# baresip/re

Hardware: AMD Instinct MI355X
Metric: GiB/s + Mpkt/s SRTP protect+unprotect, 1200B RTP pkts, device-resident (higher is better)
Workload: dtype u8

## Files before the change

re_amd/csrc/hip/k_ctr_fast.h:

```cpp
#pragma once
#include "kern_common.h"

#ifndef CTRF_BLOCK
#define CTRF_BLOCK 1024
#endif
#ifndef CTRF_BLOCK_U
#define CTRF_BLOCK_U CTRF_BLOCK
#endif
#define CTRF_BLK(PROT) ((PROT) ? CTRF_BLOCK : CTRF_BLOCK_U)
#ifndef CTRF_COAL_P
#define CTRF_COAL_P 1
#endif
#ifndef CTRF_COAL_U
#define CTRF_COAL_U 1
#endif
#ifndef CTRF_COAL_MK
#define CTRF_COAL_MK 1
#endif
#ifndef CTRF_SB_ST
#define CTRF_SB_ST 0
#endif
#ifndef CTRF_PRIO
#define CTRF_PRIO 0
#endif
#ifndef CTRF_SHAFIRST_U
#define CTRF_SHAFIRST_U 1
#endif
#ifndef CTRF_SB_BLOCKS
#define CTRF_SB_BLOCKS 0
#endif
#ifndef CTRF_SB_SHA
#define CTRF_SB_SHA 0
#endif

template <int NR, int SHIFT>
__device__ __forceinline__ void fast_ks_xor(const uint8_t *smem, uint32_t lo,
					    const uint32_t *rk,
					    const CtrKs<NR, true, true> &C,
					    int32_t blk0, uint32_t carry[4],
					    uint32_t d[16])
{
#pragma unroll
	for (int q = 0; q < SHIFT; q++)
		d[q] ^= carry[4 - SHIFT + q];
#pragma unroll
	for (int m = 0; m < 4; m++) {
		uint32_t B[4];
		C.block(smem, lo, rk, blk0 + m, B);
#pragma unroll
		for (int q = 0; q < 4; q++) {
			const int jj = SHIFT + 4 * m + q;
			if (jj < 16)
				d[jj] ^= B[q];
			else
				carry[q] = B[q];
		}
		if (m == 3 && SHIFT == 0) {
#pragma unroll
			for (int q = 0; q < 4; q++)
				carry[q] = B[q];
		}
		if (CTRF_SB_BLOCKS && (m + 1) % (CTRF_SB_BLOCKS > 0 ?
						 CTRF_SB_BLOCKS : 1) == 0 &&
		    m < 3)
			__builtin_amdgcn_sched_barrier(0);
	}
}

struct FastPkt {
	uint32_t p, off, L, hl, ssrc, ixhi, ixlo, roc;
};

template <bool RTCP = false>
__device__ __forceinline__ bool fast_pkt(const struct sgpu_compact &c,
					 uint32_t t, FastPkt &f)
{
	if (t >= c.n)
		return false;
	f.p = c.idx ? c.idx[c.base + t] : c.base + t;
	const uint64_t d = c.desc[f.p];
	const uint32_t fl = (uint32_t)(d >> 48);
	if (!(fl & SD_RUN))
		return false;
	f.off = c.pos[f.p];
	f.L = c.end[f.p] - f.off;
	const uint32_t *hw = (const uint32_t *)(c.hdr + f.p);
	f.ssrc = hw[0];
	f.hl = hw[2];
	if (RTCP) {
		const uint32_t w = (uint32_t)d;
		f.ixhi = (w & 0x7fffffffu) >> 16;
		f.ixlo = w & 0xffffu;
		f.roc = w;
		return true;
	}
	f.ixhi = (uint32_t)(d >> 16);
	f.ixlo = (uint32_t)(d & 0xffffu);
	f.roc = f.ixhi + ((fl & SD_ROC_P1) ? 1u : 0u) -
		((fl & SD_ROC_M1) ? 1u : 0u);
	return true;
}

template <int NR>
__device__ __forceinline__ const struct sgpu_comp *
fast_keys_at(const KArgs &a, uint32_t ci, uint32_t rk[4 * (NR + 1)])
{
	const struct sgpu_comp *cp = a.comps + ci;
#pragma unroll
	for (int k = 0; k < NR + 1; k++) {
		const uint4 v = *(const uint4 *)&cp->rk[4 * k];
		rk[4 * k] = v.x; rk[4 * k + 1] = v.y;
		rk[4 * k + 2] = v.z; rk[4 * k + 3] = v.w;
	}
#pragma unroll
	for (int k = 4; k < 4 * NR; k++)
		rk[k] = rot16(rk[k]);
#pragma unroll
	for (int k = 0; k < 4 * (NR + 1); k++)
		rk[k] = __builtin_amdgcn_readfirstlane(rk[k]);
	return cp;
}

template <int NR>
__device__ __forceinline__ const struct sgpu_comp *
fast_keys(const KArgs &a, uint32_t rk[4 * (NR + 1)])
{
	return fast_keys_at<NR>(
		a, __builtin_amdgcn_readfirstlane(a.c.compmap[0]), rk);
}

template <int NR>
__device__ __forceinline__ const struct sgpu_comp *
lane_keys(const KArgs &a, const FastPkt &f, uint32_t rk[4 * (NR + 1)])
{
	const struct sgpu_comp *cp = a.comps + a.c.compmap[a.c.sess[f.p]];
#pragma unroll
	for (int k = 0; k < NR + 1; k++) {
		const uint4 v = *(const uint4 *)&cp->rk[4 * k];
		rk[4 * k] = v.x; rk[4 * k + 1] = v.y;
		rk[4 * k + 2] = v.z; rk[4 * k + 3] = v.w;
	}
#pragma unroll
	for (int k = 4; k < 4 * NR; k++)
		rk[k] = rot16(rk[k]);
	return cp;
}

__device__ __forceinline__ void fast_iv(const struct sgpu_comp *cp,
					const FastPkt &f, uint32_t iv[4])
{
	const uint4 ks = *(const uint4 *)cp->k_s;
	iv[0] = ks.x;
	iv[1] = ks.y ^ bswap32(f.ssrc);
	iv[2] = ks.z ^ bswap32(f.ixhi);
	iv[3] = (ks.w ^ (bswap32(f.ixlo) >> 16)) & 0xffffu;
}

template <int NR, int SHIFT>
__device__ __forceinline__ void tail_xor_store(const uint8_t *smem,
					       uint32_t lo, const uint32_t *rk,
					       const CtrKs<NR, true, true> &C,
					       int32_t blk0, uint32_t carry[4],
					       uint32_t d[16], uint8_t *pkt,
					       uint32_t c0, uint32_t c_off,
					       uint32_t c_end)
{
	uint32_t ks[16];
	chunk_ks<NR, SHIFT>(smem, lo, rk, C, blk0, carry, ks);
#pragma unroll
	for (int jj = 0; jj < 16; jj++) {
		const uint32_t bpos = c0 + 4u * jj;
		uint32_t m = region_mask(bpos, c_off, c_end);
		asm volatile("" : "+v"(m));
		d[jj] = __builtin_amdgcn_bitop3_b32(d[jj], ks[jj], m, 0x78);
		if (bpos + 4u > c_off && bpos < c_end)
			*(uint32_t *)(pkt + bpos) = d[jj];
	}
}

template <int NR, int SHIFT, bool PROT, bool MK = false, bool RTCP = false>
__device__ __forceinline__ void ctr_fast_pkt(const KArgs &a, uint8_t *smem,
					     const FastPkt &f, uint32_t ci)
{
	uint32_t rk[4 * (NR + 1)];
	const struct sgpu_comp *cp = MK ? lane_keys<NR>(a, f, rk)
					: fast_keys_at<NR>(a, ci, rk);
	const uint32_t lo = (threadIdx.x & 31u) * 4u;
	const uint32_t lane = threadIdx.x & 63u;
	uint8_t *const arena = a.arena;
	uint8_t *const pkt = arena + f.off;
	const uint64_t pasz = a.asz - f.off;
	const uint32_t T = PROT ? 0u : __builtin_amdgcn_readfirstlane(cp->tag_len);
	const uint32_t A = f.L - T - (RTCP && !PROT ? 4u : 0u);
	const uint32_t hl = RTCP && !(f.roc >> 31) ? A : f.hl;

	uint32_t iv[4];
	fast_iv(cp, f, iv);
	CtrKs<NR, true, true> C;
	C.init(smem, lo, rk, iv);
	uint32_t h[5] = {cp->ipad[0], cp->ipad[1], cp->ipad[2], cp->ipad[3],
			 cp->ipad[4]};
	const uint64_t X = (uint64_t)f.roc << 32 | 0x80000000u;
	const uint32_t nb = (A + 4u + 9u + 63u) / 64u;
	const uint64_t bitlen = (uint64_t)(64u + A + 4u) * 8u;
	const int32_t cw4 = (int32_t)(hl >> 4);
	const uint32_t kf0 = hl < 16u ? 0u : min((hl + 63u) / 64u, nb);
	const uint32_t kf1 = max(A / 64u, kf0);
	uint32_t carry[4] = {0, 0, 0, 0};

	auto general = [&](uint32_t k) {
		const uint32_t c0 = 64u * k;
		uint32_t d[16], w[16];
#pragma unroll
		for (int g = 0; g < 4; g++) {
			uint4 v = make_uint4(0, 0, 0, 0);
			if (c0 + 16u * g < A)
				v = ld16(pkt, pasz, c0 + 16u * g);
			d[4 * g] = v.x; d[4 * g + 1] = v.y;
			d[4 * g + 2] = v.z; d[4 * g + 3] = v.w;
		}
		if (!PROT) {
#pragma unroll
			for (int jj = 0; jj < 16; jj++)
				w[jj] = msg_word(16u * k + jj, bswap32(d[jj]), A, X);
		}
		if (c0 + 64u > hl && c0 < A)
			tail_xor_store<NR, SHIFT>(smem, lo, rk, C,
						  (int32_t)(4 * k) - cw4, carry,
						  d, pkt, c0, hl, A);
		if (PROT) {
#pragma unroll
			for (int jj = 0; jj < 16; jj++)
				w[jj] = msg_word(16u * k + jj, bswap32(d[jj]), A, X);
		}
		if (k + 1 == nb) {
			w[14] = (uint32_t)(bitlen >> 32);
			w[15] = (uint32_t)bitlen;
		}
		sha1_compress(h, w);
	};

	uint32_t k = 0;
	for (; k < kf0; k++)
		general(k);

	constexpr bool COAL = MK ? CTRF_COAL_MK :
			      PROT ? CTRF_COAL_P : CTRF_COAL_U;
	uint32_t K0 = kf1, K1 = kf1;
	uint32_t qo[4];
	if constexpr (COAL) {
		qo[0] = qdpp<0x00>(f.off) + 16u * (lane & 3u);
		qo[1] = qdpp<0x55>(f.off) + 16u * (lane & 3u);
		qo[2] = qdpp<0xAA>(f.off) + 16u * (lane & 3u);
		qo[3] = qdpp<0xFF>(f.off) + 16u * (lane & 3u);
		const uint64_t act = __ballot(1);
		uint32_t a0 = max(kf0, qdpp<DPP_QXOR1>(kf0));
		a0 = max(a0, qdpp<DPP_QXOR2>(a0));
		uint32_t a1 = min(kf1, qdpp<DPP_QXOR1>(kf1));
		a1 = min(a1, qdpp<DPP_QXOR2>(a1));
		if (((act >> (lane & ~3u)) & 0xfull) == 0xfull && a0 < a1) {
			K0 = a0;
			K1 = a1;
		}
	}
	auto steady = [&](uint32_t k, auto coal) {
		constexpr bool CO = decltype(coal)::value;
		const uint32_t c0 = 64u * k;
		if (CTRF_PRIO) {
			const uint32_t q4 =
				(uint32_t)__builtin_amdgcn_readfirstlane(4u * k) /
				(uint32_t)__builtin_amdgcn_readfirstlane(nb);
			if (q4 == 0)
				__builtin_amdgcn_s_setprio(3);
			else if (q4 == 1)
				__builtin_amdgcn_s_setprio(2);
			else if (q4 == 2)
				__builtin_amdgcn_s_setprio(1);
			else
				__builtin_amdgcn_s_setprio(0);
		}
		uint32_t d[16], w[16];
		if constexpr (CO) {
			uint32_t x[4][4];
#pragma unroll
			for (int g = 0; g < 4; g++) {
				const uint4 v = *(const uint4 *)(arena + (qo[g] + c0));
				x[g][0] = v.x; x[g][1] = v.y; x[g][2] = v.z;
				x[g][3] = v.w;
			}
			quad_transpose(x, lane);
#pragma unroll
			for (int q = 0; q < 4; q++)
#pragma unroll
				for (int cc = 0; cc < 4; cc++)
					d[4 * q + cc] = x[q][cc];
		}
		else {
#pragma unroll
			for (int g = 0; g < 4; g++) {
				const uint4 v = *(const uint4 *)(pkt + c0 + 16u * g);
				d[4 * g] = v.x; d[4 * g + 1] = v.y;
				d[4 * g + 2] = v.z; d[4 * g + 3] = v.w;
			}
		}
		if (!PROT && CTRF_SHAFIRST_U) {
#pragma unroll
			for (int jj = 0; jj < 16; jj++)
				w[jj] = bswap32(d[jj]);
			sha1_compress(h, w);
			if (CTRF_SB_SHA)
				__builtin_amdgcn_sched_barrier(0);
		}
		fast_ks_xor<NR, SHIFT>(smem, lo, rk, C, (int32_t)(4 * k) - cw4,
				       carry, d);
		if constexpr (CO) {
			uint32_t x[4][4];
#pragma unroll
			for (int q = 0; q < 4; q++)
#pragma unroll
				for (int cc = 0; cc < 4; cc++)
					x[q][cc] = d[4 * q + cc];
			quad_transpose(x, lane);
#pragma unroll
			for (int g = 0; g < 4; g++)
				*(uint4 *)(arena + (qo[g] + c0)) =
					make_uint4(x[g][0], x[g][1], x[g][2],
						   x[g][3]);
		}
		else {
			if (CTRF_SB_ST)
				__builtin_amdgcn_sched_barrier(0);
#pragma unroll
			for (int g = 0; g < 4; g++)
				*(uint4 *)(pkt + c0 + 16u * g) =
					make_uint4(d[4 * g], d[4 * g + 1],
						   d[4 * g + 2], d[4 * g + 3]);
		}
		if (PROT) {
#pragma unroll
			for (int jj = 0; jj < 16; jj++)
				w[jj] = bswap32(d[jj]);
			sha1_compress(h, w);
		}
		else if (!CTRF_SHAFIRST_U) {
		}
	};
	static_assert(PROT || CTRF_SHAFIRST_U,
		      "unprotect steady chunks MAC the ciphertext first");
	for (; k < K0; k++)
		steady(k, std::false_type());
	if constexpr (COAL) {
		for (; k < K1; k++)
			steady(k, std::true_type());
		for (; k < kf1; k++)
			steady(k, std::false_type());
	}
	for (; k < nb; k++)
		general(k);

	{
		uint32_t w[16];
		w[0] = h[0]; w[1] = h[1]; w[2] = h[2]; w[3] = h[3]; w[4] = h[4];
		w[5] = 0x80000000u;
#pragma unroll
		for (int q = 6; q < 15; q++)
			w[q] = 0;
		w[15] = (64u + 20u) * 8u;
		h[0] = cp->opad[0]; h[1] = cp->opad[1]; h[2] = cp->opad[2];
		h[3] = cp->opad[3]; h[4] = cp->opad[4];
		sha1_compress(h, w);
	}
	const uint32_t tag_len = __builtin_amdgcn_readfirstlane(cp->tag_len);
	uint8_t *tp = pkt + A;
	if (PROT) {
		if (RTCP) {
			st_be32(tp, f.roc);
			tp += 4;
		}
		for (uint32_t q = 0; q < tag_len; q++)
			tp[q] = (uint8_t)(h[q >> 2] >> (24 - 8 * (q & 3)));
		return;
	}
	if (RTCP) {
		tp += 4;
		uint32_t diff = 0;
		for (uint32_t q = 0; q < tag_len; q++)
			diff |= tp[q] ^ (uint8_t)(h[q >> 2] >> (24 - 8 * (q & 3)));
		const uint8_t vd = (diff == 0 ? SV_TAG_OK : 0) | SV_CIPHERED;
		if (!(vd & SV_TAG_OK))
			atomicAdd(a.c.nfail, 1u);
		if (a.verdict)
			a.verdict[f.p] = vd;
		return;
	}
	uint32_t diff = 0;
	for (uint32_t q = 0; q < tag_len; q++)
		diff |= tp[q] ^ (uint8_t)(h[q >> 2] >> (24 - 8 * (q & 3)));
	if (a.c.save)
		a.c.save[f.p] = (uint32_t)tp[0] | (uint32_t)tp[1] << 8 |
				(uint32_t)tp[2] << 16 | (uint32_t)tp[3] << 24;
	st_be32(tp, f.roc);
	const uint8_t vd = (diff == 0 ? SV_TAG_OK : 0) | SV_CIPHERED;
	if (!(vd & SV_TAG_OK)) {
		const uint32_t q = atomicAdd(a.c.nfail, 1u);
		if (a.c.flist)
			a.c.flist[q] = f.p;
	}
	if (a.verdict)
		a.verdict[f.p] = vd;
}

#ifndef CTRF_FILL_LOOP
#define CTRF_FILL_LOOP 0
#endif
template <int NR, int SHIFT, bool PROT, bool MK = false, bool RTCP = false>
__device__ __forceinline__ void ctr_fast_body(const KArgs &a, uint8_t *smem)
{
	if (CTRF_FILL_LOOP || blockDim.x != 1024u)
		tt4_fill(smem, a.t0);
	else
		tt4_fill_b1024(smem, a.t0);
	__syncthreads();
	FastPkt f;
	if (!fast_pkt<RTCP>(a.c, blockIdx.x * blockDim.x + threadIdx.x, f))
		return;
	ctr_fast_pkt<NR, SHIFT, PROT, MK, RTCP>(
		a, smem, f,
		MK ? 0u : __builtin_amdgcn_readfirstlane(a.c.compmap[0]));
}

template <int NR, bool MK = false>
__global__ void __launch_bounds__(256)
k_ctr_refix_list(const KArgs a)
{
	__shared__ __attribute__((aligned(16))) uint8_t smem[TT4_BYTES];
	const uint32_t nf = *(volatile const uint32_t *)a.c.nfail;
	if (blockIdx.x >= nf)
		return;
	tt4_fill(smem, a.t0);
	__syncthreads();
	uint32_t rk[4 * (NR + 1)];
	const struct sgpu_comp *cp = MK ? a.comps : fast_keys<NR>(a, rk);
	const uint32_t lo = (threadIdx.x & 31u) * 4u;
	for (uint32_t q = blockIdx.x; q < nf; q += gridDim.x) {
		const uint32_t p = a.c.flist[q];
		FastPkt f;
		if (!MK && !fast_pkt(a.c, p - a.c.base, f))
			continue;
		if (MK) {
			const uint64_t d = a.c.desc[p];
			const uint32_t fl = (uint32_t)(d >> 48);
			if (!(fl & SD_RUN))
				continue;
			f.p = p;
			f.off = a.c.pos[p];
			f.L = a.c.end[p] - f.off;
			const uint32_t *hw = (const uint32_t *)(a.c.hdr + p);
			f.ssrc = hw[0];
			f.hl = hw[2];
			f.ixhi = (uint32_t)(d >> 16);
			f.ixlo = (uint32_t)(d & 0xffffu);
			f.roc = f.ixhi + ((fl & SD_ROC_P1) ? 1u : 0u) -
				((fl & SD_ROC_M1) ? 1u : 0u);
			const uint32_t ci = __builtin_amdgcn_readfirstlane(
				a.c.compmap[a.c.sess[p]]);
			cp = a.comps + ci;
#pragma unroll
			for (int k = 0; k < NR + 1; k++) {
				const uint4 v = *(const uint4 *)&cp->rk[4 * k];
				rk[4 * k] = v.x; rk[4 * k + 1] = v.y;
				rk[4 * k + 2] = v.z; rk[4 * k + 3] = v.w;
			}
#pragma unroll
			for (int k = 4; k < 4 * NR; k++)
				rk[k] = rot16(rk[k]);
#pragma unroll
			for (int k = 0; k < 4 * (NR + 1); k++)
				rk[k] = __builtin_amdgcn_readfirstlane(rk[k]);
		}
		const uint32_t T = __builtin_amdgcn_readfirstlane(cp->tag_len);
		uint8_t *pkt = a.arena + f.off;
		const uint32_t A = f.L - T;
		uint32_t iv[4];
		fast_iv(cp, f, iv);
		CtrKs<NR, true, true> C;
		C.init(smem, lo, rk, iv);
		for (uint32_t b = threadIdx.x; f.hl + 16u * b < A;
		     b += blockDim.x) {
			uint32_t ks[4];
			C.block(smem, lo, rk, (int32_t)b, ks);
			const uint32_t p0 = f.hl + 16u * b;
#pragma unroll
			for (int w = 0; w < 4; w++) {
				const uint32_t bp = p0 + 4u * w;
				if (bp >= A)
					break;
				if (A - bp >= 4u) {
					uint32_t *wp = (uint32_t *)(pkt + bp);
					*wp = *wp ^ ks[w];
				}
				else {
					for (uint32_t k = 0; k < A - bp; k++)
						pkt[bp + k] ^= (uint8_t)(ks[w] >>
									 (8 * k));
				}
			}
		}
		if (threadIdx.x == 0)
			a.verdict[p] &= (uint8_t)~SV_CIPHERED;
	}
}

template <int NR, int SHIFT>
__device__ __forceinline__ void ctr_refix_body(const KArgs &a, uint8_t *smem)
{
	if (*(volatile const uint32_t *)a.c.nfail == 0)
		return;
	FastPkt f;
	const bool live = fast_pkt(a.c, blockIdx.x * blockDim.x + threadIdx.x,
				   f);
	const uint8_t vd = live ? a.verdict[f.p] : (uint8_t)SV_TAG_OK;
	const bool need = !(vd & SV_TAG_OK) && (vd & SV_CIPHERED);
	if (!__syncthreads_or(need))
		return;
	tt4_fill(smem, a.t0);
	__syncthreads();
	if (!need)
		return;
	uint32_t rk[4 * (NR + 1)];
	const struct sgpu_comp *cp = fast_keys<NR>(a, rk);
	const uint32_t lo = (threadIdx.x & 31u) * 4u;
	uint8_t *pkt = a.arena + f.off;
	const uint64_t pasz = a.asz - f.off;
	const uint32_t A = f.L - cp->tag_len;
	const int32_t cw4 = (int32_t)(f.hl >> 4);
	uint32_t iv[4];
	fast_iv(cp, f, iv);
	CtrKs<NR, true, true> C;
	C.init(smem, lo, rk, iv);
	uint32_t carry[4] = {0, 0, 0, 0};
	for (uint32_t k = 0; 64u * k < A; k++) {
		const uint32_t c0 = 64u * k;
		if (c0 + 64u <= f.hl)
			continue;
		uint32_t d[16];
#pragma unroll
		for (int g = 0; g < 4; g++) {
			uint4 v = make_uint4(0, 0, 0, 0);
			if (c0 + 16u * g < A)
				v = ld16(pkt, pasz, c0 + 16u * g);
			d[4 * g] = v.x; d[4 * g + 1] = v.y;
			d[4 * g + 2] = v.z; d[4 * g + 3] = v.w;
		}
		tail_xor_store<NR, SHIFT>(smem, lo, rk, C,
					  (int32_t)(4 * k) - cw4, carry, d, pkt,
					  c0, f.hl, A);
	}
	a.verdict[f.p] = vd & (uint8_t)~SV_CIPHERED;
}

__device__ __forceinline__ int fast_class(const KArgs &a)
{
	prof_guard(a);
	if (a.c.gfail && *a.c.gfail)
		return -1;
	const uint32_t *g = a.c.guard;
	return !g[3] ? 3 : !g[0] ? 0 : !g[1] ? 1 : !g[2] ? 2 : -1;
}

template <int NR, bool PROT>
__global__ void
__attribute__((amdgpu_flat_work_group_size(1, CTRF_BLK(PROT))))
__attribute__((amdgpu_waves_per_eu(CTRF_BLK(PROT) / 256, 8)))
k_ctr_fast_any(const KArgs a)
{
	__shared__ __attribute__((aligned(16))) uint8_t smem[TT4_BYTES];
	switch (fast_class(a)) {
	case 0: ctr_fast_body<NR, 0, PROT>(a, smem); break;
	case 1: ctr_fast_body<NR, 1, PROT>(a, smem); break;
	case 2: ctr_fast_body<NR, 2, PROT>(a, smem); break;
	case 3: ctr_fast_body<NR, 3, PROT>(a, smem); break;
	default: break;
	}
}

#ifndef CTRF_MK_BLOCK
#define CTRF_MK_BLOCK 768
#endif
template <int NR, bool PROT>
__global__ void
__attribute__((amdgpu_flat_work_group_size(1, CTRF_MK_BLOCK)))
__attribute__((amdgpu_waves_per_eu(CTRF_MK_BLOCK / 256, 8)))
k_ctr_fast_mk(const KArgs a)
{
	__shared__ __attribute__((aligned(16))) uint8_t smem[TT4_BYTES];
	switch (fast_class(a)) {
	case 0: ctr_fast_body<NR, 0, PROT, true>(a, smem); break;
	case 1: ctr_fast_body<NR, 1, PROT, true>(a, smem); break;
	case 2: ctr_fast_body<NR, 2, PROT, true>(a, smem); break;
	case 3: ctr_fast_body<NR, 3, PROT, true>(a, smem); break;
	default: break;
	}
}

template <int NR, bool PROT>
__global__ void
__attribute__((amdgpu_flat_work_group_size(1, CTRF_BLK(PROT))))
__attribute__((amdgpu_waves_per_eu(CTRF_BLK(PROT) / 256, 8)))
k_ctr_fast_rtcp(const KArgs a)
{
	__shared__ __attribute__((aligned(16))) uint8_t smem[TT4_BYTES];
	prof_guard(a);
	if (*a.c.guard)
		return;
	ctr_fast_body<NR, 2, PROT, false, true>(a, smem);
}

template <int NR>
__global__ void
__attribute__((amdgpu_flat_work_group_size(1, CTRF_BLOCK)))
__attribute__((amdgpu_waves_per_eu(CTRF_BLOCK / 256, 8)))
k_ctr_fast_refix(const KArgs a)
{
	__shared__ __attribute__((aligned(16))) uint8_t smem[TT4_BYTES];
	switch (fast_class(a)) {
	case 0: ctr_refix_body<NR, 0>(a, smem); break;
	case 1: ctr_refix_body<NR, 1>(a, smem); break;
	case 2: ctr_refix_body<NR, 2>(a, smem); break;
	case 3: ctr_refix_body<NR, 3>(a, smem); break;
	default: break;
	}
}
```

re_amd/csrc/hip/kern_common.h:

```cpp
#pragma once
#include <hip/hip_runtime.h>
#include <errno.h>
#include <stdint.h>
#include "../srtpgpu.h"
#include "dev_common.h"

#define KBLOCK 256
#define CTR_BLOCK 512
#define CTR_BLOCK_MAX 768


__device__ __forceinline__ uint4 ld16(const uint8_t *arena, uint64_t asz,
				      uint64_t a)
{
	if (a + 16 <= asz)
		return *(const uint4 *)(arena + a);
	uint4 r = make_uint4(0, 0, 0, 0);
	if (a + 4 <= asz)  r.x = *(const uint32_t *)(arena + a);
	if (a + 8 <= asz)  r.y = *(const uint32_t *)(arena + a + 4);
	if (a + 12 <= asz) r.z = *(const uint32_t *)(arena + a + 8);
	return r;
}

__device__ __forceinline__ void st_partial(uint8_t *p, uint32_t v, uint32_t n)
{
	if (n >= 2) {
		*(uint16_t *)p = (uint16_t)v;
		if (n == 3)
			p[2] = (uint8_t)(v >> 16);
	}
	else if (n == 1) {
		p[0] = (uint8_t)v;
	}
}

__device__ __forceinline__ void st_be32(uint8_t *p, uint32_t v)
{
	p[0] = (uint8_t)(v >> 24);
	p[1] = (uint8_t)(v >> 16);
	p[2] = (uint8_t)(v >> 8);
	p[3] = (uint8_t)v;
}

template <int NR, bool T4>
__device__ __forceinline__ void ctr_block(const uint8_t *smem, uint32_t lo,
					  const uint32_t *rk, const uint32_t iv[4],
					  int32_t b, uint32_t ks[4])
{
	uint64_t c = ((uint64_t)bswap32(iv[2]) << 32 | bswap32(iv[3])) +
		     (uint64_t)(int64_t)b;
	uint32_t s0 = iv[0], s1 = iv[1];
	uint32_t s2 = bswap32((uint32_t)(c >> 32));
	uint32_t s3 = bswap32((uint32_t)c);
	if (T4) {
		const Tt4 T = {smem, lo, lo | 0x10000u};
		s0 ^= rk[0]; s1 ^= rk[1]; s2 ^= rk[2]; s3 ^= rk[3];
		aes4_rounds<NR, 1>(T, rk, s0, s1, s2, s3);
	}
	else {
		aes_block<NR>(smem, lo, rk, s0, s1, s2, s3);
	}
	ks[0] = s0; ks[1] = s1; ks[2] = s2; ks[3] = s3;
}

#ifndef CTR_B15
#define CTR_B15 1
#endif

template <int NR, bool CACHED, bool T4 = false, bool B8 = false>
struct CtrKs {
	uint32_t t0, t1, t2, t3c;
	uint32_t A0, P0, A1, P1;
	uint32_t R0, C1a, C1b, C2, C3a, C3b;

	__device__ __forceinline__ void init(const uint8_t *smem, uint32_t lo,
					     const uint32_t *rk,
					     const uint32_t iv[4])
	{
		t0 = iv[0] ^ rk[0];
		t1 = iv[1] ^ rk[1];
		t2 = iv[2] ^ rk[2];
		t3c = iv[3] ^ rk[3];
		if (!CACHED)
			return;
		const uint32_t *k1 = rk + 4, *k2 = rk + 8;
		if (T4) {
			const Tt4 T = {smem, lo, lo | 0x10000u};
			A0 = xor3(T.t0(t0), T.t1(t1), T.t2(t2)) ^ k1[0];
			A1 = xor3(T.t0(t1), T.t1(t2), T.t3(t0)) ^ k1[1];
			const uint32_t S2 = xor3(xor3(T.t0(t2), T.t1(t3c), T.t2(t0)),
						 T.t3(t1), k1[2]);
			const uint32_t S3 = xor3(xor3(T.t0(t3c), T.t1(t0), T.t2(t1)),
						 T.t3(t2), k1[3]);
			R0 = xor3(T.t2(S2), T.t3(S3), k2[0]);
			C1a = xor3(T.t1(S2), T.t2(S3), k2[1]);
			C2 = xor3(T.t0(S2), T.t1(S3), k2[2]);
			C3a = xor3(T.t0(S3), T.t3(S2), k2[3]);
#if CTR_B15
			const uint32_t s1 = A1 ^ T.t2(t3c);
			R0 ^= T.t1(s1);
			C1a ^= T.t0(s1);
			C2 ^= T.t3(s1);
			C3a ^= T.t2(s1);
			A1 = TT_ADDRH(t3c, 3, lo | 0x10000u) + 128u;
#endif
			return;
		}
		A0 = lds_u32(smem, TT_ADDR(t0, 0, lo)) ^
		     lds_u32(smem, TT_ADDR(t1, 1, lo) + 128);
		P0 = lds_u32(smem, TT_ADDR(t2, 2, lo)) ^ k1[0];
		A1 = lds_u32(smem, TT_ADDR(t1, 0, lo)) ^
		     lds_u32(smem, TT_ADDR(t2, 1, lo) + 128);
		P1 = lds_u32(smem, TT_ADDR(t0, 3, lo) + 128) ^ k1[1];
		const uint32_t S2 = xor3(lds_u32(smem, TT_ADDR(t2, 0, lo)),
					 lds_u32(smem, TT_ADDR(t3c, 1, lo) + 128),
					 rot16(xor3(lds_u32(smem, TT_ADDR(t0, 2, lo)),
						    lds_u32(smem, TT_ADDR(t1, 3, lo) + 128),
						    k1[2])));
		const uint32_t S3 = xor3(lds_u32(smem, TT_ADDR(t3c, 0, lo)),
					 lds_u32(smem, TT_ADDR(t0, 1, lo) + 128),
					 rot16(xor3(lds_u32(smem, TT_ADDR(t1, 2, lo)),
						    lds_u32(smem, TT_ADDR(t2, 3, lo) + 128),
						    k1[3])));
		R0 = rot16(xor3(lds_u32(smem, TT_ADDR(S2, 2, lo)),
				lds_u32(smem, TT_ADDR(S3, 3, lo) + 128), k2[0]));
		C1a = lds_u32(smem, TT_ADDR(S2, 1, lo) + 128);
		C1b = lds_u32(smem, TT_ADDR(S3, 2, lo)) ^ k2[1];
		C2 = lds_u32(smem, TT_ADDR(S2, 0, lo)) ^
		     lds_u32(smem, TT_ADDR(S3, 1, lo) + 128);
		C3a = lds_u32(smem, TT_ADDR(S3, 0, lo));
		C3b = lds_u32(smem, TT_ADDR(S2, 3, lo) + 128) ^ k2[3];
		if (B8) {
			const uint32_t s1 = A1 ^ rot16(P1 ^ lds_u32(smem,
						TT_ADDR(t3c, 2, lo)));
			R0 ^= lds_u32(smem, TT_ADDR(s1, 1, lo) + 128);
			C1a ^= lds_u32(smem, TT_ADDR(s1, 0, lo));
			C2 ^= rot16(lds_u32(smem, TT_ADDR(s1, 3, lo) + 128) ^
				    k2[2]);
			C3a ^= rot16(lds_u32(smem, TT_ADDR(s1, 2, lo)) ^ C3b);
		}
	}

	__device__ __forceinline__ void block(const uint8_t *smem, uint32_t lo,
					      const uint32_t *rk, int32_t b,
					      uint32_t ks[4]) const
	{
		if (!CACHED) {
			const uint32_t iv[4] = {t0 ^ rk[0], t1 ^ rk[1],
						t2 ^ rk[2], t3c ^ rk[3]};
			ctr_block<NR, T4>(smem, lo, rk, iv, b, ks);
			return;
		}
		if (T4 && CTR_B15) {
			const Tt4 T = {smem, lo, lo | 0x10000u};
			const uint32_t s0 = A0 ^ lds_u32(smem, A1 ^
					(((uint32_t)b & 255u) << 8));
			uint32_t r0 = T.t0(s0) ^ R0;
			uint32_t r1 = T.t3(s0) ^ C1a;
			uint32_t r2 = T.t2(s0) ^ C2;
			uint32_t r3 = T.t1(s0) ^ C3a;
			aes4_rounds<NR, 3>(T, rk, r0, r1, r2, r3);
			ks[0] = r0; ks[1] = r1; ks[2] = r2; ks[3] = r3;
			return;
		}
		const uint32_t t3 = t3c ^ bswap32((uint32_t)b);
		if (T4) {
			const Tt4 T = {smem, lo, lo | 0x10000u};
			const uint32_t s0 = A0 ^ T.t3(t3);
			const uint32_t s1 = A1 ^ T.t2(t3);
			uint32_t r0 = xor3(T.t0(s0), T.t1(s1), R0);
			uint32_t r1 = xor3(T.t0(s1), T.t3(s0), C1a);
			uint32_t r2 = xor3(T.t2(s0), T.t3(s1), C2);
			uint32_t r3 = xor3(T.t1(s0), T.t2(s1), C3a);
			aes4_rounds<NR, 3>(T, rk, r0, r1, r2, r3);
			ks[0] = r0; ks[1] = r1; ks[2] = r2; ks[3] = r3;
			return;
		}
		if (B8) {
			const uint32_t t3b = t3c ^ ((uint32_t)b << 24);
			const uint32_t s0 = A0 ^ rot16(P0 ^ lds_u32(smem,
						TT_ADDR(t3b, 3, lo) + 128));
			uint32_t r0 = lds_u32(smem, TT_ADDR(s0, 0, lo)) ^ R0;
			uint32_t r1 = C1a ^ rot16(C1b ^ lds_u32(smem,
						TT_ADDR(s0, 3, lo) + 128));
			uint32_t r2 = C2 ^ rot16(lds_u32(smem,
						TT_ADDR(s0, 2, lo)));
			uint32_t r3 = C3a ^ lds_u32(smem,
						   TT_ADDR(s0, 1, lo) + 128);
			aes_rounds<NR, 3>(smem, lo, rk, r0, r1, r2, r3);
			ks[0] = r0; ks[1] = r1; ks[2] = r2; ks[3] = r3;
			return;
		}
		const uint32_t s0 = A0 ^ rot16(P0 ^ lds_u32(smem,
					TT_ADDR(t3, 3, lo) + 128));
		const uint32_t s1 = A1 ^ rot16(P1 ^ lds_u32(smem,
					TT_ADDR(t3, 2, lo)));
		const uint32_t *k2 = rk + 8;
		uint32_t r0 = xor3(lds_u32(smem, TT_ADDR(s0, 0, lo)),
				   lds_u32(smem, TT_ADDR(s1, 1, lo) + 128), R0);
		uint32_t r1 = xor3(lds_u32(smem, TT_ADDR(s1, 0, lo)), C1a,
				   rot16(C1b ^ lds_u32(smem,
					TT_ADDR(s0, 3, lo) + 128)));
		uint32_t r2 = C2 ^ rot16(xor3(lds_u32(smem, TT_ADDR(s0, 2, lo)),
					      lds_u32(smem, TT_ADDR(s1, 3, lo) + 128),
					      k2[2]));
		uint32_t r3 = xor3(C3a, lds_u32(smem, TT_ADDR(s0, 1, lo) + 128),
				   rot16(lds_u32(smem, TT_ADDR(s1, 2, lo)) ^ C3b));
		aes_rounds<NR, 3>(smem, lo, rk, r0, r1, r2, r3);
		ks[0] = r0; ks[1] = r1; ks[2] = r2; ks[3] = r3;
	}
};

__device__ __forceinline__ uint32_t msg_word(uint32_t gw, uint32_t data_be,
					     uint32_t A, uint64_t X)
{
	uint32_t aw = A >> 2, u = A & 3;
	if (gw < aw)
		return data_be;
	if (gw == aw)
		return (data_be & (uint32_t)(0xFFFFFFFF00000000ull >> (8 * u))) |
		       (uint32_t)(X >> (32 + 8 * u));
	if (gw == aw + 1)
		return (uint32_t)(X >> (8 * u));
	return 0;
}


struct KArgs {
	const uint32_t *t0;
	uint8_t *arena;
	uint64_t asz;
	const struct sgpu_job *jobs;
	uint32_t njobs;
	const struct sgpu_comp *comps;
	uint8_t *verdict;
	uint32_t *save;
	struct sgpu_compact c;
	int nocipher;
	uint32_t *done_cnt;
	uint32_t *done_flag;
	uint32_t done_seq;
	uint32_t *pguard;
	uint32_t pguard_n;
};

__device__ __forceinline__ void prof_guard(const KArgs &a)
{
	if (a.pguard && a.c.guard && blockIdx.x == 0 && threadIdx.x == 0) {
		const bool gf = a.c.gfail && *a.c.gfail;
		for (uint32_t q = 0; q < a.pguard_n; q++)
			a.pguard[q] = gf ? 1u : a.c.guard[q];
	}
}

template <int MODE, bool PROT>
__device__ __forceinline__ bool rtcp_job(const KArgs &a,
					 const struct sgpu_compact &c,
					 uint32_t p, uint64_t d, uint8_t vd,
					 struct sgpu_job &j)
{
	const uint32_t comp = c.compmap[0];
	const struct sgpu_comp *cp = a.comps + comp;
	const uint32_t off = c.pos[p];
	const uint32_t L = c.end[p] - off;
	const uint32_t ix = (uint32_t)d & 0x7fffffffu;
	const uint32_t E = ((uint32_t)d >> 31) & 1u;
	const uint32_t T = cp->tag_len;
	const bool hmac = (cp->flags & 2u) != 0;
	j.off = off;
	j.comp = comp;
	j.ssrc = ((const uint32_t *)(c.hdr + p))[0];
	j.ixhi = ix >> 16;
	j.ixlo = ix & 0xffffu;
	j.trailer = E << 31 | ix;
	j.c_off = 8;
	j.t_off = 0;
	if (PROT) {
		if (MODE == SGPU_MODE_CTR) {
			j.flags = SJ_PROTECT | SJ_STORE_TRAIL |
				  (E ? SJ_CIPHER : 0u) |
				  (hmac ? (SJ_HMAC | SJ_TRAILER) : 0u);
			j.c_len = L - 8u;
			j.t_off = L;
			j.a_len = L;
			j.tag_off = L + 4u;
		}
		else {
			j.flags = SJ_PROTECT | SJ_GCM | SJ_TRAILER |
				  SJ_STORE_TRAIL | (E ? SJ_CIPHER : 0u);
			j.a_len = E ? 8u : L;
			j.c_len = E ? L - 8u : 0u;
			j.tag_off = L;
			j.t_off = L + 16u;
		}
		return true;
	}
	if (MODE == SGPU_MODE_CTR) {
		const uint32_t tag_start = L - T, eix_start = L - T - 4u;
		j.c_len = eix_start - 8u;
		j.a_len = tag_start;
		j.tag_off = tag_start;
		if (c.undo)
			j.flags = (vd & SV_CIPHERED) ? SJ_CIPHER : 0u;
		else
			j.flags = SJ_HMAC | ((E && (cp->flags & 1u)) ?
					     (SJ_CIPHER | SJ_CIPHER_IF_OK) : 0u);
	}
	else {
		const uint32_t tag_start = L - 4u - 16u;
		j.tag_off = tag_start;
		j.a_len = E ? 8u : tag_start;
		j.c_len = E ? tag_start - 8u : 0u;
		j.flags = c.undo ? (SJ_GCM | SJ_CIPHER | SJ_UNDO)
				 : (SJ_GCM | SJ_TRAILER | (E ? SJ_CIPHER : 0u));
	}
	return true;
}

template <bool COMPACT, int MODE, bool PROT>
__device__ __forceinline__ bool get_job(const KArgs &a, uint32_t t,
					struct sgpu_job &j, uint32_t &slot)
{
	if (!COMPACT) {
		if (t >= a.njobs)
			return false;
		j = a.jobs[t];
		slot = t;
		return true;
	}
	const struct sgpu_compact &c = a.c;
	if (t >= c.n)
		return false;
	if (c.guard && *c.guard)
		return false;
	const uint32_t p = c.idx ? c.idx[c.base + t] : c.base + t;
	slot = p;
	const uint64_t d = c.desc[p];
	const uint32_t fl = (uint32_t)(d >> 48);
	j.flags = SJ_SKIP;
	j.comp = 0;
	if (!(fl & SD_RUN))
		return true;
	uint8_t vd = 0;
	if (c.undo) {
		vd = a.verdict[p];
		if (MODE == SGPU_MODE_GCM && !(vd & SV_CIPHERED))
			return true;
	}
	if (c.rtcp)
		return rtcp_job<MODE, PROT>(a, c, p, d, vd, j);
	const uint32_t comp = c.compmap[c.sess ? c.sess[p] : 0u];
	const uint32_t off = c.pos[p];
	const uint32_t L = c.end[p] - off;
	const uint32_t *hw = (const uint32_t *)(c.hdr + p);
	const uint32_t ssrc = hw[0], hl = hw[2];
	const uint32_t ixhi = (uint32_t)(d >> 16);
	j.off = off;
	j.comp = comp;
	j.ssrc = ssrc;
	j.ixhi = ixhi;
	j.ixlo = (uint32_t)(d & 0xffffu);
	j.trailer = ixhi + ((fl & SD_ROC_P1) ? 1u : 0u) -
		    ((fl & SD_ROC_M1) ? 1u : 0u);
	j.t_off = 0;
	j.c_off = hl;
	if (MODE == SGPU_MODE_CTR) {
		if (PROT) {
			j.flags = SJ_PROTECT | SJ_CIPHER | SJ_HMAC | SJ_TRAILER;
			j.a_len = L;
			j.c_len = L - hl;
			j.tag_off = L;
		}
		else {
			const uint32_t T = a.comps[comp].tag_len;
			j.a_len = L - T;
			j.tag_off = L - T;
			j.c_len = L - T - hl;
			if (c.undo)
				j.flags = (vd & SV_CIPHERED) ? SJ_CIPHER : 0u;
			else
				j.flags = SJ_HMAC | SJ_TRAILER | SJ_ROC_AT_TAG |
					  ((fl & SD_CIPHER) ?
					   (SJ_CIPHER | SJ_CIPHER_IF_OK) : 0u);
		}
	}
	else {
		j.a_len = hl;
		if (PROT) {
			j.flags = SJ_PROTECT | SJ_CIPHER | SJ_GCM;
			j.c_len = L - hl;
			j.tag_off = L;
		}
		else {
			j.flags = c.undo ? (SJ_GCM | SJ_CIPHER | SJ_UNDO)
					 : (SJ_GCM | SJ_CIPHER);
			j.c_len = L - 16u - hl;
			j.tag_off = L - 16u;
		}
	}
	return true;
}

__device__ __forceinline__ uint32_t region_mask(uint32_t bpos, uint32_t c_off,
						uint32_t c_end)
{
	const uint32_t nbytes = (bpos >= c_off && bpos < c_end) ?
				min(c_end - bpos, 4u) : 0u;
	return (uint32_t)((1ull << (8 * nbytes)) - 1ull);
}

template <int NR, int SHIFT, bool MASKED, bool CACHED, bool T4>
__device__ __forceinline__ void ks_xor(const uint8_t *smem, uint32_t lo,
				       const uint32_t *rk,
				       const CtrKs<NR, CACHED, T4> &C,
				       int32_t blk0, uint32_t carry[4],
				       uint32_t d[16], uint32_t c0 = 0,
				       uint32_t c_off = 0, uint32_t c_end = 0)
{
#define KS_MASK(jj) (MASKED ? region_mask(c0 + 4u * (jj), c_off, c_end) \
			    : 0xffffffffu)
#pragma unroll
	for (int q = 0; q < SHIFT; q++)
		d[q] ^= carry[4 - SHIFT + q] & KS_MASK(q);
#pragma unroll
	for (int m = 0; m < 4; m++) {
		uint32_t B[4];
		C.block(smem, lo, rk, blk0 + m, B);
#pragma unroll
		for (int q = 0; q < 4; q++) {
			const int jj = SHIFT + 4 * m + q;
			if (jj < 16)
				d[jj] ^= B[q] & KS_MASK(jj);
			else
				carry[q] = B[q];
		}
		if (m == 3 && SHIFT == 0) {
#pragma unroll
			for (int q = 0; q < 4; q++)
				carry[q] = B[q];
		}
	}
#undef KS_MASK
}

template <int NR, int SHIFT, bool CACHED, bool T4>
__device__ __forceinline__ void ks_xor_km(const uint8_t *smem, uint32_t lo,
					  const uint32_t *rk,
					  const CtrKs<NR, CACHED, T4> &C,
					  int32_t blk0, uint32_t carry[4],
					  uint32_t d[16], uint32_t km)
{
#pragma unroll
	for (int q = 0; q < SHIFT; q++)
		d[q] = __builtin_amdgcn_bitop3_b32(d[q], carry[4 - SHIFT + q], km,
						   0x78);
#pragma unroll
	for (int m = 0; m < 4; m++) {
		uint32_t B[4];
		C.block(smem, lo, rk, blk0 + m, B);
#pragma unroll
		for (int q = 0; q < 4; q++) {
			const int jj = SHIFT + 4 * m + q;
			if (jj < 16)
				d[jj] = __builtin_amdgcn_bitop3_b32(d[jj], B[q], km,
								   0x78);
			else
				carry[q] = B[q];
		}
		if (m == 3 && SHIFT == 0) {
#pragma unroll
			for (int q = 0; q < 4; q++)
				carry[q] = B[q];
		}
	}
}

template <int NR, int SHIFT, bool CACHED, bool T4>
__device__ __forceinline__ void chunk_ks(const uint8_t *smem, uint32_t lo,
					 const uint32_t *rk,
					 const CtrKs<NR, CACHED, T4> &C,
					 int32_t blk0, uint32_t carry[4],
					 uint32_t ks[16])
{
#pragma unroll
	for (int q = 0; q < SHIFT; q++)
		ks[q] = carry[4 - SHIFT + q];
#pragma unroll
	for (int m = 0; m < 4; m++) {
		uint32_t B[4];
		C.block(smem, lo, rk, blk0 + m, B);
#pragma unroll
		for (int q = 0; q < 4; q++) {
			const int jj = SHIFT + 4 * m + q;
			if (jj < 16)
				ks[jj] = B[q];
			else
				carry[q] = B[q];
		}
	}
}

#define DPP_QXOR1 0xB1
#define DPP_QXOR2 0x4E

template <int CTRL>
__device__ __forceinline__ uint32_t qdpp(uint32_t v)
{
	return (uint32_t)__builtin_amdgcn_mov_dpp((int)v, CTRL, 0xf, 0xf, false);
}

__device__ __forceinline__ void quad_transpose(uint32_t x[4][4], uint32_t lane)
{
	const uint32_t m0 = 0u - (lane & 1u), m1 = 0u - ((lane >> 1) & 1u);
#pragma unroll
	for (int c = 0; c < 4; c++) {
#pragma unroll
		for (int r = 0; r < 4; r += 2) {
			const uint32_t t0 = qdpp<DPP_QXOR1>(x[r][c]);
			const uint32_t t1 = qdpp<DPP_QXOR1>(x[r + 1][c]);
			x[r + 1][c] = sha_ch(m0, x[r + 1][c], t0);
			x[r][c] = sha_ch(m0, t1, x[r][c]);
		}
#pragma unroll
		for (int r = 0; r < 2; r++) {
			const uint32_t t0 = qdpp<DPP_QXOR2>(x[r][c]);
			const uint32_t t2 = qdpp<DPP_QXOR2>(x[r + 2][c]);
			x[r + 2][c] = sha_ch(m1, x[r + 2][c], t0);
			x[r][c] = sha_ch(m1, t2, x[r][c]);
		}
	}
}

__device__ __forceinline__ void quad_offsets(uint64_t off, uint32_t lane,
					     uint64_t qb[4])
{
	const uint32_t lo = (uint32_t)off, hi = (uint32_t)(off >> 32);
	const uint32_t l4[4] = {qdpp<0x00>(lo), qdpp<0x55>(lo),
				qdpp<0xAA>(lo), qdpp<0xFF>(lo)};
	const uint32_t h4[4] = {qdpp<0x00>(hi), qdpp<0x55>(hi),
				qdpp<0xAA>(hi), qdpp<0xFF>(hi)};
#pragma unroll
	for (int g = 0; g < 4; g++)
		qb[g] = ((uint64_t)h4[g] << 32 | l4[g]) + 16u * (lane & 3u);
}

__device__ __forceinline__ void quad_load(const uint8_t *arena,
					  const uint64_t qb[4], uint32_t c0,
					  uint32_t lane, uint32_t d[16])
{
	uint32_t x[4][4];
#pragma unroll
	for (int g = 0; g < 4; g++) {
		const uint4 v = *(const uint4 *)(arena + qb[g] + c0);
		x[g][0] = v.x; x[g][1] = v.y; x[g][2] = v.z; x[g][3] = v.w;
	}
	quad_transpose(x, lane);
#pragma unroll
	for (int q = 0; q < 4; q++)
#pragma unroll
		for (int c = 0; c < 4; c++)
			d[4 * q + c] = x[q][c];
}

__device__ __forceinline__ void quad_store(uint8_t *arena, const uint64_t qb[4],
					   uint32_t c0, uint32_t lane,
					   const uint32_t s[16])
{
	uint32_t x[4][4];
#pragma unroll
	for (int q = 0; q < 4; q++)
#pragma unroll
		for (int c = 0; c < 4; c++)
			x[q][c] = s[4 * q + c];
	quad_transpose(x, lane);
#pragma unroll
	for (int g = 0; g < 4; g++)
		*(uint4 *)(arena + qb[g] + c0) =
			make_uint4(x[g][0], x[g][1], x[g][2], x[g][3]);
}

__device__ __forceinline__ void store_region_exact(uint8_t *pkt, uint32_t c0,
						   const uint32_t d[16],
						   uint32_t c_off, uint32_t c_end)
{
	volatile uint8_t *vp = pkt;
#pragma unroll
	for (int jj = 0; jj < 16; jj++) {
		const uint32_t bpos = c0 + 4u * jj;
		if (bpos >= c_off && bpos < c_end) {
			const uint32_t nbytes = min(c_end - bpos, 4u);
			if (nbytes == 4)
				*(volatile uint32_t *)(vp + bpos) = d[jj];
			else
				for (uint32_t z = 0; z < nbytes; z++)
					vp[bpos + z] = (uint8_t)(d[jj] >> (8 * z));
		}
	}
}

__device__ __forceinline__ void store_region(uint8_t *pkt, uint32_t c0,
					     const uint32_t d[16],
					     uint32_t c_off, uint32_t c_end)
{
#pragma unroll
	for (int jj = 0; jj < 16; jj++) {
		const uint32_t bpos = c0 + 4u * jj;
		if (bpos >= c_off && bpos < c_end) {
			const uint32_t nbytes = min(c_end - bpos, 4u);
			if (nbytes == 4)
				*(uint32_t *)(pkt + bpos) = d[jj];
			else
				st_partial(pkt + bpos, d[jj], nbytes);
		}
	}
}

typedef void (*kfn_t)(const KArgs);

#define SGPU_SMALL_MAX_BYTES 2048
int small_launch(uint8_t *arena, uint64_t arena_size,
		 const struct sgpu_job *jobs, uint32_t njobs, uint8_t *verdict,
		 uint32_t *save, const struct sgpu_comp *comps,
		 const uint32_t *t0, int prot, uint32_t *done_cnt,
		 uint32_t *done_flag, uint32_t done_seq, void *stream);

int small_srv_launch(const struct sgpu_comp *comps, const uint32_t *t0,
		     struct sgpu_srv_mb *mb, struct sgpu_srv_bc *bc,
		     uint32_t grid, uint32_t linger_us, uint32_t life_us,
		     uint32_t *done_cnt, uint32_t *done_flag, void *stream);

unsigned sgpu_ctr_block(bool uni, int prot);
kfn_t sgpu_pick_ctr10(bool compact, bool uni, int shift, int prot);
kfn_t sgpu_pick_ctr10_coop(int prot);
kfn_t sgpu_pick_gcm_coop(int nr);
kfn_t sgpu_pick_ctr14_coop(int prot);
kfn_t sgpu_pick_ctr14(bool compact, bool uni, int shift, int prot);
kfn_t sgpu_pick_ctr10_any(bool uni, int prot);
kfn_t sgpu_pick_ctr14_any(bool uni, int prot);
kfn_t sgpu_pick_gcm(bool compact, bool uni, int nr, int prot);
kfn_t sgpu_pick_ctr10_fast(int prot, int refix);
kfn_t sgpu_pick_ctr14_fast(int prot, int refix);
unsigned sgpu_ctr_fast_block(int prot);
kfn_t sgpu_pick_ctr10_fast_mk(int prot);
kfn_t sgpu_pick_ctr14_fast_mk(int prot);
kfn_t sgpu_pick_ctr10_fast_rtcp(int prot);
kfn_t sgpu_pick_ctr14_fast_rtcp(int prot);
unsigned sgpu_ctr_fast_mk_block(void);
unsigned sgpu_gcm_block(bool uni);
```

Measured before the change: 484.6.

## Transpose coalesced packet chunks across rows with permlane swaps instead of quads

Adds a new default transpose mode for the coalesced CTR+SHA1 steady loop. Groups of four lanes spaced 16 apart, rather than adjacent quad lanes, cooperate on loads, using the permlane32/permlane16 swap builtins for the transpose, offset broadcast and min/max reductions. An alternative DPP v_cndmask-based quad transpose is also added but is not the default. The aim is to cut the instruction count of the quad_transpose DPP shuffles in the hot loop, at the cost of a different lane-to-packet grouping and therefore a different memory access pattern.

```diff
diff --git a/re_amd/csrc/hip/k_ctr_fast.h b/re_amd/csrc/hip/k_ctr_fast.h
--- a/re_amd/csrc/hip/k_ctr_fast.h
+++ b/re_amd/csrc/hip/k_ctr_fast.h
@@ -16,6 +16,12 @@
 #endif
 #ifndef CTRF_COAL_MK
 #define CTRF_COAL_MK 1
+#endif
+#ifndef CTRF_XPOSE
+#define CTRF_XPOSE 1
+#endif
+#ifndef CTRF_XPOSE_MK
+#define CTRF_XPOSE_MK 0
 #endif
 #ifndef CTRF_SB_ST
 #define CTRF_SB_ST 0
@@ -248,7 +254,17 @@
 			      PROT ? CTRF_COAL_P : CTRF_COAL_U;
 	uint32_t K0 = kf1, K1 = kf1;
 	uint32_t qo[4];
-	if constexpr (COAL) {
+	constexpr int XP = MK ? CTRF_XPOSE_MK : CTRF_XPOSE;
+	if constexpr (COAL && XP == 1) {
+		row_offsets(f.off, lane, qo);
+		const uint64_t act = __ballot(1);
+		const uint32_t a0 = row_max(kf0), a1 = row_min(kf1);
+		if (row_all(act, lane) && a0 < a1) {
+			K0 = a0;
+			K1 = a1;
+		}
+	}
+	else if constexpr (COAL) {
 		qo[0] = qdpp<0x00>(f.off) + 16u * (lane & 3u);
 		qo[1] = qdpp<0x55>(f.off) + 16u * (lane & 3u);
 		qo[2] = qdpp<0xAA>(f.off) + 16u * (lane & 3u);
@@ -288,7 +304,12 @@
 				x[g][0] = v.x; x[g][1] = v.y; x[g][2] = v.z;
 				x[g][3] = v.w;
 			}
-			quad_transpose(x, lane);
+			if constexpr (XP == 1)
+				row_transpose(x);
+			else if constexpr (XP == 2)
+				quad_transpose_cnd(x);
+			else
+				quad_transpose(x, lane);
 #pragma unroll
 			for (int q = 0; q < 4; q++)
 #pragma unroll
@@ -320,7 +341,12 @@
 #pragma unroll
 				for (int cc = 0; cc < 4; cc++)
 					x[q][cc] = d[4 * q + cc];
-			quad_transpose(x, lane);
+			if constexpr (XP == 1)
+				row_transpose(x);
+			else if constexpr (XP == 2)
+				quad_transpose_cnd(x);
+			else
+				quad_transpose(x, lane);
 #pragma unroll
 			for (int g = 0; g < 4; g++)
 				*(uint4 *)(arena + (qo[g] + c0)) =
diff --git a/re_amd/csrc/hip/kern_common.h b/re_amd/csrc/hip/kern_common.h
--- a/re_amd/csrc/hip/kern_common.h
+++ b/re_amd/csrc/hip/kern_common.h
@@ -531,6 +531,93 @@
 	}
 }
 
+template <uint32_t MASK, bool XOR2>
+__device__ __forceinline__ void qcnd8(const uint32_t a[8], const uint32_t b[8],
+				      uint32_t o[8])
+{
+#define QCND_(N, QP)                                                       \
+	"v_cndmask_b32_dpp %" #N ", %" QCND_A_(N) ", %" QCND_B_(N)             \
+	", vcc quad_perm:" QP " row_mask:0xf bank_mask:0xf\n\t"
+#define QCND_A_(N) QCND_A##N
+#define QCND_B_(N) QCND_B##N
+#define QCND_A0 "8"
+#define QCND_A1 "9"
+#define QCND_A2 "10"
+#define QCND_A3 "11"
+#define QCND_A4 "12"
+#define QCND_A5 "13"
+#define QCND_A6 "14"
+#define QCND_A7 "15"
+#define QCND_B0 "16"
+#define QCND_B1 "17"
+#define QCND_B2 "18"
+#define QCND_B3 "19"
+#define QCND_B4 "20"
+#define QCND_B5 "21"
+#define QCND_B6 "22"
+#define QCND_B7 "23"
+#define QCND8_(QP)                                                         \
+	asm("s_mov_b32 vcc_lo, %24\n\ts_mov_b32 vcc_hi, %24\n\t"               \
+	    QCND_(0, QP) QCND_(1, QP) QCND_(2, QP) QCND_(3, QP)                \
+	    QCND_(4, QP) QCND_(5, QP) QCND_(6, QP) QCND_(7, QP)                \
+	    : "=&v"(o[0]), "=&v"(o[1]), "=&v"(o[2]), "=&v"(o[3]),              \
+	      "=&v"(o[4]), "=&v"(o[5]), "=&v"(o[6]), "=&v"(o[7])               \
+	    : "v"(a[0]), "v"(a[1]), "v"(a[2]), "v"(a[3]), "v"(a[4]),           \
+	      "v"(a[5]), "v"(a[6]), "v"(a[7]), "v"(b[0]), "v"(b[1]),           \
+	      "v"(b[2]), "v"(b[3]), "v"(b[4]), "v"(b[5]), "v"(b[6]),           \
+	      "v"(b[7]), "n"(MASK)                                             \
+	    : "vcc")
+	if constexpr (XOR2)
+		QCND8_("[2,3,0,1]");
+	else
+		QCND8_("[1,0,3,2]");
+#undef QCND8_
+#undef QCND_
+#undef QCND_A_
+#undef QCND_B_
+}
+
+__device__ __forceinline__ void quad_transpose_cnd(uint32_t x[4][4])
+{
+	uint32_t lo[8], hi[8], n[4][4];
+#pragma unroll
+	for (int c = 0; c < 4; c++) {
+		lo[c] = x[0][c]; lo[4 + c] = x[2][c];
+		hi[c] = x[1][c]; hi[4 + c] = x[3][c];
+	}
+	{
+		uint32_t o[8];
+		qcnd8<0xAAAAAAAAu, false>(lo, hi, o);
+#pragma unroll
+		for (int c = 0; c < 4; c++) {
+			n[1][c] = o[c]; n[3][c] = o[4 + c];
+		}
+		qcnd8<0x55555555u, false>(hi, lo, o);
+#pragma unroll
+		for (int c = 0; c < 4; c++) {
+			n[0][c] = o[c]; n[2][c] = o[4 + c];
+		}
+	}
+#pragma unroll
+	for (int c = 0; c < 4; c++) {
+		lo[c] = n[0][c]; lo[4 + c] = n[1][c];
+		hi[c] = n[2][c]; hi[4 + c] = n[3][c];
+	}
+	{
+		uint32_t o[8];
+		qcnd8<0xCCCCCCCCu, true>(lo, hi, o);
+#pragma unroll
+		for (int c = 0; c < 4; c++) {
+			x[2][c] = o[c]; x[3][c] = o[4 + c];
+		}
+		qcnd8<0x33333333u, true>(hi, lo, o);
+#pragma unroll
+		for (int c = 0; c < 4; c++) {
+			x[0][c] = o[c]; x[1][c] = o[4 + c];
+		}
+	}
+}
+
 __device__ __forceinline__ void quad_offsets(uint64_t off, uint32_t lane,
 					     uint64_t qb[4])
 {
@@ -577,6 +664,66 @@
 	for (int g = 0; g < 4; g++)
 		*(uint4 *)(arena + qb[g] + c0) =
 			make_uint4(x[g][0], x[g][1], x[g][2], x[g][3]);
+}
+
+__device__ __forceinline__ void row_swap32(uint32_t &a, uint32_t &b)
+{
+	const auto v = __builtin_amdgcn_permlane32_swap(a, b, false, false);
+	a = v[0]; b = v[1];
+}
+
+__device__ __forceinline__ void row_swap16(uint32_t &a, uint32_t &b)
+{
+	const auto v = __builtin_amdgcn_permlane16_swap(a, b, false, false);
+	a = v[0]; b = v[1];
+}
+
+__device__ __forceinline__ void row_transpose(uint32_t x[4][4])
+{
+#pragma unroll
+	for (int c = 0; c < 4; c++) {
+		row_swap32(x[0][c], x[2][c]);
+		row_swap32(x[1][c], x[3][c]);
+		row_swap16(x[0][c], x[1][c]);
+		row_swap16(x[2][c], x[3][c]);
+	}
+}
+
+__device__ __forceinline__ void row_offsets(uint32_t off, uint32_t lane,
+					    uint32_t qo[4])
+{
+	qo[0] = qo[1] = qo[2] = qo[3] = off;
+	row_swap32(qo[0], qo[2]);
+	row_swap32(qo[1], qo[3]);
+	row_swap16(qo[0], qo[1]);
+	row_swap16(qo[2], qo[3]);
+#pragma unroll
+	for (int g = 0; g < 4; g++)
+		qo[g] += 16u * (lane >> 4);
+}
+
+__device__ __forceinline__ uint32_t row_max(uint32_t v)
+{
+	uint32_t a = v, b = v;
+	row_swap32(a, b);
+	a = b = max(a, b);
+	row_swap16(a, b);
+	return max(a, b);
+}
+
+__device__ __forceinline__ uint32_t row_min(uint32_t v)
+{
+	uint32_t a = v, b = v;
+	row_swap32(a, b);
+	a = b = min(a, b);
+	row_swap16(a, b);
+	return min(a, b);
+}
+
+__device__ __forceinline__ bool row_all(uint64_t act, uint32_t lane)
+{
+	const uint64_t m = 0x0001000100010001ull;
+	return ((act >> (lane & 15u)) & m) == m;
 }
 
 __device__ __forceinline__ void store_region_exact(uint8_t *pkt, uint32_t c0,
```

Result: no change. 486.3 (median of 3 runs) (+0.4%).
